# fredxia/openr

Measured on AMD Instinct MI355X. Metric: all-sources SPF solves/sec + GTEPS, 10k-node fabric, 1/2/4/8 MI355X, higher is better.
Workload: dtype u32; 1 GPU; fabric_full numOfSws=10000 (RoutingBenchmarkUtils.cpp:247-400, every pod wired); nodes=9976, directed_up_edges=232512, next_hop_rows=sliced

## Files before the change

### openr_amd/csrc/plan_host.cpp

```cpp
#include "plan_host.h"

#include <algorithm>
#include <map>
#include <numeric>
#include <utility>

namespace spfi {

PlanRows plan_rows(const GraphHost& g, const uint32_t* srcs, uint32_t n_src) {
  PlanRows r;
  r.row_of.assign(g.N, kInf);
  std::vector<uint32_t>& row_of = r.row_of;
  r.distinct = true;
  for (uint32_t i = 0; i < n_src; ++i) {
    if (row_of[srcs[i]] != kInf) r.distinct = false;
    else row_of[srcs[i]] = i;
  }
  bool closed = r.distinct;
  for (uint32_t i = 0; i < n_src && closed; ++i) {
    const uint32_t s = srcs[i];
    for (uint32_t j = g.nb_ptr[s]; j < g.nb_ptr[s + 1]; ++j) {
      const uint32_t x = g.nb_id[j];
      if (!g.ovl[x] && row_of[x] == kInf) {
        closed = false;
// ... 31 lines not shown
  l.nh_off.resize(n_src);
  l.words.resize(n_src);
  uint64_t off = 0;
  for (uint32_t i = 0; i < n_src; ++i) {
    const uint32_t k = g.nb_ptr[srcs[i] + 1] - g.nb_ptr[srcs[i]];
    l.words[i] = k;
    l.nh_off[i] = off;
    off += (uint64_t)k * (g.pitch / 32);
    l.wmax = std::max(l.wmax, (k + 31) / 32);
  }
  l.nh_total = off;
  return l;
}

NbRows plan_nb_rows(const GraphHost& g, const uint32_t* srcs, uint32_t n_src,
                    const std::vector<uint32_t>& row_of, uint64_t stride, size_t rows) {
  NbRows nb;
  nb.nb_row_off.resize(n_src);
  nb.nb_drained.assign(n_src, 0);
  const uint32_t dead = stride ? (uint32_t)(rows * stride) : kInf;
  nb.dead = dead;
  std::vector<uint32_t>& nb_row = nb.nb_row;
  for (uint32_t i = 0; i < n_src; ++i) {
    nb.nb_row_off[i] = (uint32_t)nb_row.size();
    for (uint32_t e = g.nb_ptr[srcs[i]]; e < g.nb_ptr[srcs[i] + 1]; ++e) {
      const uint32_t x = g.nb_id[e];
      const bool dr = g.ovl[x] != 0;
      nb_row.push_back(dr ? dead : stride ? (uint32_t)(row_of[x] * stride) : row_of[x]);
      nb.nb_drained[i] += dr;
    }
    const size_t k = nb_row.size() - nb.nb_row_off[i];
    nb_row.resize(nb.nb_row_off[i] + (k + 7) / 8 * 8 + 8, dead);
  }
  return nb;
}

ClassRows plan_class_rows(const GraphHost& g, const std::vector<uint32_t>& closure) {
  ClassRows cr;
  const std::vector<uint16_t>& cls = g.qt.cls;
  cr.fwd.assign(g.qt.n_cls, 0);
  for (uint32_t v = 0; v < g.N; ++v)
    if (!g.ovl[v]) cr.fwd[cls[v]] = 1;
  std::vector<uint32_t> src_of(g.qt.n_cls, kInf);
  cr.crow_of.resize(closure.size());
  for (size_t r = 0; r < closure.size(); ++r) {
    uint32_t& k = src_of[cls[closure[r]]];
    if (k == kInf) {
      k = (uint32_t)cr.csrc.size();
      cr.csrc.push_back(closure[r]);
    }
    cr.crow_of[r] = k;
  }
  return cr;
}

XcdLists plan_xcd_lists(const std::vector<uint32_t>& words, uint32_t runs) {
  XcdLists x;
  const uint32_t n_src = (uint32_t)words.size();
  if (runs == 0) {
    for (uint32_t i = 0; i < n_src; ++i) x.list[i % 8].push_back(i);
  } else {
    uint64_t total = 0, load[8] = {};
    for (uint32_t i = 0; i < n_src; ++i) total += words[i] + 1;
    const uint64_t target = std::max<uint64_t>(1, total / (8ull * runs));
    for (uint32_t i = 0; i < n_src;) {
      uint32_t e = i;
      uint64_t w = 0;
      while (e < n_src && w < target) w += words[e++] + 1;
      const int g = (int)(std::min_element(load, load + 8) - load);
      load[g] += w;
      for (uint32_t t = i; t < e; ++t) x.list[g].push_back(t);
      i = e;
    }
  }
  size_t most = 0;
  for (const auto& l : x.list) most = std::max(most, l.size());
  x.slot.assign(most * 8, kInf);
  for (int g = 0; g < 8; ++g)
    for (size_t t = 0; t < x.list[g].size(); ++t) x.slot[t * 8 + g] = x.list[g][t];
  x.slots = x.slot.size();
  if (x.slot.empty()) x.slot.push_back(kInf);
  return x;
}

uint32_t plan_sliced_unit(const std::vector<uint32_t>& words, uint32_t chunks, uint32_t n_cu) {
  uint64_t matches = 0;
  for (uint32_t k : words) matches += (uint64_t)k * chunks;
  return (uint32_t)std::min<uint64_t>(kSlUnit, std::max<uint64_t>(16, matches / (16ull * n_cu) / 8 * 8));
}

SlicedUnits plan_sliced_units(const std::vector<uint32_t> (&list)[8], const std::vector<uint32_t>& words,
                              const NbRows& nb, uint32_t chunks, uint32_t unit, int group) {
  SlicedUnits s;
  std::vector<uint32_t>& units = s.units;
  std::vector<uint32_t>& gtab = s.gtab;
  s.unit_off.assign(9, 0);
  const uint32_t dead = nb.dead;
  for (int g = 0; g < 8; ++g) {
    s.unit_off[g] = (uint32_t)(units.size() / 4);
    std::map<uint32_t, std::vector<uint8_t>> taken;
    std::map<std::vector<uint32_t>, std::vector<std::pair<uint32_t, uint32_t>>> shared;
    if (group) {
      std::map<std::vector<uint32_t>, std::vector<uint32_t>> seg;
      for (uint32_t i : list[g]) {
        const uint32_t k = words[i];
        if (!k) continue;
// ... 186 lines not shown
```

### openr_amd/csrc/plan_host.h

```cpp
#pragma once
#include <cstddef>
#include <cstdint>
#include <vector>

#include "graph_host.h"

namespace spfi {

constexpr uint32_t kEcmpRunsPerXcd = 64;
constexpr uint32_t kSlSlots = 8;
constexpr uint32_t kSlSat = 254;
constexpr uint32_t kSlGroup = 8;
constexpr uint32_t kSlSeg = 4;
constexpr uint32_t kSlUnit = 512;

struct PlanRows {
  bool distinct = false, direct = false;
  std::vector<uint32_t> closure, row_of, req_rows;
};
PlanRows plan_rows(const GraphHost& g, const uint32_t* srcs, uint32_t n_src);

struct NhLayout {
  std::vector<uint32_t> words;
  std::vector<uint64_t> nh_off;
  uint64_t nh_total = 0;
  uint32_t wmax = 1;
};
NhLayout plan_nh_layout(const GraphHost& g, const uint32_t* srcs, uint32_t n_src);

struct NbRows {
  std::vector<uint32_t> nb_row, nb_row_off, nb_drained;
  uint32_t dead = kInf;
};
NbRows plan_nb_rows(const GraphHost& g, const uint32_t* srcs, uint32_t n_src,
                    const std::vector<uint32_t>& row_of, uint64_t stride, size_t rows);

struct XcdLists {
  std::vector<uint32_t> list[8];
  std::vector<uint32_t> slot;
  size_t slots = 0;
};
XcdLists plan_xcd_lists(const std::vector<uint32_t>& words, uint32_t runs);

struct SlicedUnits {
  std::vector<uint32_t> units, unit_off, gtab;
  uint32_t max_xcd_units = 0;
};
SlicedUnits plan_sliced_units(const std::vector<uint32_t> (&list)[8], const std::vector<uint32_t>& words,
                              const NbRows& nb, uint32_t chunks, uint32_t unit, int group);
uint32_t plan_sliced_unit(const std::vector<uint32_t>& words, uint32_t chunks, uint32_t n_cu);

struct ClassRows {
  std::vector<uint32_t> csrc, crow_of;
  std::vector<uint8_t> fwd;
};
ClassRows plan_class_rows(const GraphHost& g, const std::vector<uint32_t>& closure);

struct DepthCache {
  std::vector<uint32_t> ecc;
  uint64_t ecc_epoch = ~0ull;
  uint32_t dbound = 0;
  uint64_t dbound_epoch = ~0ull;
  struct Memo {
    uint64_t sell_ver;
    std::vector<uint8_t> ovl;
    uint32_t dbound;
  };
  std::vector<Memo> memo;
};
const std::vector<uint32_t>& ecc_estimate(const GraphHost& g, DepthCache* m);
std::vector<uint32_t> plan_depth_order(const std::vector<uint32_t>& closure, const std::vector<uint32_t>& ecc);
uint32_t depth_bound(const GraphHost& g, DepthCache* m);

}
```

### openr_amd/csrc/spf_engine.hip

```cpp
#include <hip/hip_runtime.h>

#include <algorithm>
#include <chrono>
#include <cstdarg>
#include <cstdio>
#include <cstdlib>
#include <cstring>
#include <map>
#include <memory>
#include <mutex>
#include <numeric>
#include <string>
#include <type_traits>
#include <unordered_map>
#include <vector>

#include "engine_internal.h"
#include "wave_ops.h"

namespace spfi {

thread_local std::string g_err;

spf_status fail(spf_ctx* c, spf_status st, const char* fmt, ...) {
// ... 961 lines not shown
      uint32_t k[kQChunk];
#pragma unroll
      for (uint32_t j = 0; j < kQChunk; ++j) k[j] = vcol[j * q_nvp + r];
      uint64_t acc = 0;
#pragma unroll
      for (uint32_t j = 0; j < kQChunk; ++j) acc |= CFc[k[j]];
      if (acc) atomicOr(reinterpret_cast<unsigned long long*>(&QAc[vrow[r]]), acc);
    }
    for (uint32_t t = tid; t <= q_nc; t += kMsThreads) {
      CFn[t] = 0;
      QAn[t] = 0;
    }
    __syncthreads();
    uint64_t any = 0;
    for (uint32_t t0 = tid - lane; t0 < q_nc; t0 += kMsThreads) {
      const uint32_t t = t0 + lane;
      uint64_t nx = 0;
      if (t < q_nc) {
        const uint64_t v = VIS[t];
        nx = QAc[t] & ~v;
        if (nx) {
          VIS[t] = v | nx;
          if (fw[t]) CFn[t] = nx;
        }
      }
      any |= nx;
      for (uint64_t m = wave_or64(nx); m; m &= m - 1) {
        const uint32_t s = __ffsll((unsigned long long)m) - 1;
        if ((nx >> s) & 1ull) Dc[(size_t)(row0 + s) * cpitch + t] = (uint16_t)(L + 1);
      }
    }
    if (any) flag[L % 3] = 1;
    if (tid == 0) flag[(L + 1) % 3] = 0;
    __syncthreads();
    if (!flag[L % 3]) {
      last = L;
      break;
    }
  }
  if (tid == 0) atomicMax(maxd, last);
  for (uint32_t t0 = tid - lane; t0 < q_nc; t0 += kMsThreads) {
    const uint32_t t = t0 + lane;
    const uint64_t miss = t < q_nc ? ~VIS[t] & all : 0ull;
    for (uint64_t m = wave_or64(miss); m; m &= m - 1) {
      const uint32_t s = __ffsll((unsigned long long)m) - 1;
      if ((miss >> s) & 1ull) Dc[(size_t)(row0 + s) * cpitch + t] = 0xFFFFu;
    }
  }
  const uint32_t pw = cpitch - q_nc;
  for (uint32_t t = tid; t < nb * pw; t += kMsThreads)
    Dc[(size_t)(row0 + t / pw) * cpitch + q_nc + t % pw] = 0xFFFFu;
}

constexpr uint32_t kExThreads = 256;
constexpr uint32_t kExNodes = 4 * kExThreads;
constexpr uint32_t kExRows = 8;
__global__ __launch_bounds__(kExThreads) void expand_rows_kernel(
    const uint16_t* __restrict__ Dc, uint32_t cpitch, const uint32_t* __restrict__ crow_of,
    const uint32_t* __restrict__ closure, uint32_t rows, uint32_t rows_per,
    const uint16_t* __restrict__ q_cls, uint32_t q_nc, uint32_t N, uint32_t pitch, uint32_t npitch,
    uint32_t* __restrict__ D, uint8_t* __restrict__ Dn, uint32_t* __restrict__ S,
    const uint32_t* __restrict__ maxd) {
  extern __shared__ __attribute__((aligned(16))) unsigned char smem[];
  uint4* const T = reinterpret_cast<uint4*>(smem);
  uint32_t* const list = reinterpret_cast<uint32_t*>(T + kExNodes + 1);
  uint32_t* const cnt = list + kExNodes + 1;
  uint32_t* const map = cnt + 3;
  constexpr uint32_t kEmpty = 0xFFFFFFFFu, kClaimed = 0xFFFFFFFEu;

  const uint32_t tid = threadIdx.x, lane = tid & 63;
  const uint32_t cbase = blockIdx.x * kExNodes, v0 = cbase + tid * 4;
  const uint32_t r_begin = blockIdx.y * rows_per, r_end = min(rows, r_begin + rows_per);
  const uint32_t md = *maxd;
  const uint32_t P = (S && md < kSlSat) ? 32u - __clz(md + 1u) : 0u;
  const uint32_t wpm = pitch / 32;

  for (uint32_t t = tid; t < q_nc; t += kExThreads) map[t] = kEmpty;
  if (tid == 0) {
    *cnt = 1;
    T[0] = make_uint4(~0u, ~0u, ~0u, ~0u);
  }
  __syncthreads();
  uint32_t cl[4];
#pragma unroll
  for (int k = 0; k < 4; ++k) {
    cl[k] = v0 + k < N ? q_cls[v0 + k] : kEmpty;
    if (cl[k] != kEmpty && atomicCAS(&map[cl[k]], kEmpty, kClaimed) == kEmpty) {
      const uint32_t id = atomicAdd(cnt, 1u);
      list[id] = cl[k];
      map[cl[k]] = id;
    }
  }
  __syncthreads();
  const uint32_t n_loc = *cnt;
#pragma unroll
  for (int k = 0; k < 4; ++k) cl[k] = cl[k] != kEmpty ? map[cl[k]] : 0u;

  const uint32_t w = v0 / 32, pb = lane & 7u, nsh = 4u * pb;
  const bool d_live = D && v0 < pitch, n_live = Dn && v0 < npitch, s_live = pb < P && w < wpm;
  for (uint32_t r0 = r_begin; r0 < r_end; r0 += kExRows) {
    __syncthreads();
    for (uint32_t lc = 1 + tid; lc < n_loc; lc += kExThreads) {
      const uint32_t gc = list[lc];
      uint32_t x[kExRows];
#pragma unroll
      for (uint32_t j = 0; j < kExRows; ++j)
        x[j] = r0 + j < r_end ? Dc[(size_t)crow_of[r0 + j] * cpitch + gc] : 0xFFFFu;
      T[lc] = make_uint4(x[0] | x[1] << 16, x[2] | x[3] << 16, x[4] | x[5] << 16, x[6] | x[7] << 16);
    }
    __syncthreads();
    uint4 t[4];
#pragma unroll
    for (int k = 0; k < 4; ++k) t[k] = T[cl[k]];
#pragma unroll
    for (uint32_t j = 0; j < kExRows; ++j) {
      const uint32_t r = r0 + j;
      if (r >= r_end) break;
      uint32_t d[4];
#pragma unroll
      for (int k = 0; k < 4; ++k) {
        const uint32_t pair = j / 2 == 0 ? t[k].x : j / 2 == 1 ? t[k].y : j / 2 == 2 ? t[k].z : t[k].w;
        d[k] = (uint32_t)(int32_t)(int16_t)(pair >> (16 * (j & 1)));
      }
      const uint32_t self = closure[r] - v0;
      if (closure[r] - cbase < kExNodes) {
#pragma unroll
        for (int k = 0; k < 4; ++k) d[k] = self == (uint32_t)k ? 0u : d[k];
      }
      if (d_live) {
        typedef uint32_t u32x4 __attribute__((ext_vector_type(4)));
        const u32x4 o = {d[0], d[1], d[2], d[3]};
        __builtin_nontemporal_store(o, reinterpret_cast<u32x4*>(D + (size_t)r * pitch + v0));
      }
      if (n_live) {
        uint32_t b = 0;
#pragma unroll
        for (int k = 0; k < 4; ++k) b |= (d[k] == kInf ? 0xFFu : min(d[k], 254u)) << (8 * k);
        __builtin_nontemporal_store(b, reinterpret_cast<uint32_t*>(Dn + (size_t)r * npitch + v0));
      }
      if (P) {
        uint32_t mine = 0;
        for (uint32_t b = 0; b < P; ++b) {
          uint32_t nib = ((d[0] >> b) & 1u) | ((d[1] >> b) & 1u) << 1 | ((d[2] >> b) & 1u) << 2 |
                         ((d[3] >> b) & 1u) << 3;
          nib <<= nsh;
          nib |= (uint32_t)__builtin_amdgcn_update_dpp(0u, nib, 0xB1, 0xf, 0xf, true);
          nib |= (uint32_t)__builtin_amdgcn_update_dpp(0u, nib, 0x4E, 0xf, 0xf, true);
          nib |= (uint32_t)__builtin_amdgcn_update_dpp(0u, nib, 0x104, 0xf, 0x5, true) |
                 (uint32_t)__builtin_amdgcn_update_dpp(0u, nib, 0x114, 0xf, 0xa, true);
          mine = pb == b ? nib : mine;
        }
        if (s_live) S[(size_t)r * kSlSlots * wpm + (size_t)w * P + pb] = mine;
      }
    }
  }
}

template <int P>
struct Planes {
  uint32_t v[P];
};

typedef uint32_t u32x3 __attribute__((ext_vector_type(3)));
typedef uint32_t u32x4 __attribute__((ext_vector_type(4)));

template <int N>
__device__ __forceinline__ void bload(uint32_t* d, __amdgpu_buffer_rsrc_t r, uint32_t voff,
                                      uint32_t soff) {
  if constexpr (N >= 4) {
    const u32x4 a = __builtin_amdgcn_raw_buffer_load_b128(r, (int)voff, (int)soff, 0);
    d[0] = a.x, d[1] = a.y, d[2] = a.z, d[3] = a.w;
    if constexpr (N > 4) bload<N - 4>(d + 4, r, voff + 16, soff);
  } else if constexpr (N == 3) {
    const u32x3 a = __builtin_amdgcn_raw_buffer_load_b96(r, (int)voff, (int)soff, 0);
    d[0] = a.x, d[1] = a.y, d[2] = a.z;
  } else if constexpr (N == 2) {
    const u32x2 a = __builtin_amdgcn_raw_buffer_load_b64(r, (int)voff, (int)soff, 0);
    d[0] = a.x, d[1] = a.y;
  } else {
    d[0] = __builtin_amdgcn_raw_buffer_load_b32(r, (int)voff, (int)soff, 0);
  }
}

#ifndef SPF_SL_STORE_AUX
#define SPF_SL_STORE_AUX 2
#endif
constexpr int kSlStoreAux = SPF_SL_STORE_AUX;
template <int P, bool WEIGHTED = false, int U = (P <= 4 ? 4 : 2)>
__device__ __forceinline__ void sliced_pass(__amdgpu_buffer_rsrc_t rs, __amdgpu_buffer_rsrc_t ro,
                                            uint32_t wpm, uint32_t srow,
                                            const uint32_t* __restrict__ offs, uint32_t k,
                                            uint32_t jb, uint32_t w, bool live,
                                            const uint32_t* __restrict__ wts = nullptr) {
  const uint32_t wpb = w * P * 4;
  Planes<P> sv;
  bload<P>(sv.v, rs, wpb, srow * kSlSlots * wpm * 4);
  uint32_t t[P];
  uint32_t ones = ~0u, zeros = ~0u, borrow = ~0u;
#pragma unroll
  for (int b = 0; b < P; ++b) {
    const uint32_t x = sv.v[b];
    ones &= x;
    zeros &= ~x;
    t[b] = WEIGHTED ? x : x ^ borrow;
    borrow &= ~x;
  }
  const uint32_t valid = ~(ones | zeros);
// ... 326 lines not shown
      if (PASS) {
        const unsigned long long key = ((unsigned long long)du << 32) | r;
        uint32_t p = base + n;
        while (p > base) {
          const unsigned long long pk = pred_key[p - 1];
          if (pk < key) break;
          pred_key[p] = pk;
          pred_edge[p] = (uint32_t)pk;
          --p;
        }
        pred_key[p] = key;
        pred_edge[p] = r;
      }
      ++n;
    }
  }
  if (!PASS) cnt_or_ptr[v] = n;
}


size_t sssp_lds_bytes(uint32_t N, uint32_t pitch, uint32_t big, bool q16) {
  const uint32_t bm_words = (N + 31) / 32;
  size_t b = 4ull * pitch + 4ull * bm_words + 4ull * C_NWORDS + 4ull * big;
  b += (q16 ? 2ull : 4ull) * N;
  return (b + 15) & ~size_t(15);
}

size_t msbfs_lds_bytes(uint32_t N, bool db = false) {
  return 8ull * (N + 1) * (db ? 2 : 1) + 4ull * (4 * kMsBatch + 5);
}

bool ms_double_buffer(const spf_ctx* c) {
  const char* e = std::getenv("SPF_MSBFS_DB");
  if (e && e[0] == '0') return false;
  const size_t n_col = c->sell_ptr.back();
  return msbfs_lds_bytes(c->N) + 2ull * n_col > kMaxLds && msbfs_lds_bytes(c->N, true) <= kMaxLds;
}

size_t msbfs_q_lds_bytes(uint32_t N, uint32_t n_cls, uint32_t n_vrow) {
  const size_t nvp = (n_vrow + 7u) & ~7u;
  return 32ull * (n_cls + 1) + 2ull * (1 + kQChunk) * nvp + 4ull * (4 * kMsBatch + 5) + ((N + 3u) & ~3u);
}

bool quotient_allowed(const spf_ctx* c) {
  if (c->N > kMsMaxNodes || ms_own(c->N) > (uint32_t)kQMaxOwn) return false;
  const char* e = std::getenv("SPF_QUOTIENT");
  return !(e && e[0] == '0');
}

size_t class_bfs_lds_bytes(uint32_t n_cls, uint32_t n_vrow) {
  const size_t nvp = (n_vrow + 7u) & ~7u, nc1 = (n_cls + 2u) & ~1u;
  return 40ull * nc1 + 2ull * (1 + kQChunk) * nvp + 16 + ((n_cls + 15u) & ~15u);
}
size_t expand_lds_bytes(uint32_t n_cls) { return 20ull * (kExNodes + 1) + 12 + 4ull * n_cls + 16; }

uint32_t spread_batch(const spf_ctx* c, uint32_t rows, uint32_t full) {
  const uint32_t rounds = (rows + full * c->n_cu - 1) / (full * c->n_cu);
  return std::min<uint32_t>(full, (rows + rounds * c->n_cu - 1) / (rounds * c->n_cu));
}

uint32_t ms_batch(const spf_ctx* c, uint32_t rows, bool knob = true) {
  if (const char* e = knob ? std::getenv("SPF_MSBFS_BATCH") : nullptr) {
    const int b = atoi(e);
    if (b >= 1 && b <= (int)kMsBatch) return (uint32_t)b;
  }
  return spread_batch(c, rows, kMsBatch);
}

uint32_t planes_batch(const spf_ctx* c, uint32_t rows, bool ordered) {
  return ordered ? kPlBatch : spread_batch(c, rows, kPlBatch);
}

size_t planes_lds_bytes(uint32_t own) { return 8ull * own * kMsThreads + 4ull * (kPlBatch + 4); }

}

namespace spfi {

bool use_quotient(const spf_ctx* c) {
  const spf_ctx::Quotient& q = c->qt;
  if (!quotient_allowed(c) || q.stale || q.n_cls == 0 || 2 * q.n_edge > c->nb_id.size()) return false;
  return msbfs_q_lds_bytes(c->N, q.n_cls, q.n_vrow) <= kMaxLds;
}

bool plan_has_narrow(const spf_plan* p) {
  return !p->exact && !p->big && p->narrow && !p->sdirect && (p->d_Dn.p || p->cls);
}

bool use_planes(const spf_ctx* c) {
  if (c->N > 10 * (uint32_t)kMsThreads || c->sell4.empty()) return false;
  if (const char* e = std::getenv("SPF_MSBFS")) return e[0] == 'p';
  return c->sell_ptr.back() <= 8ull * c->N;
}

spf_status launch_sssp(spf_ctx* c, const uint32_t* rows_src, uint32_t rows, bool hop,
                       const uint32_t* ign, uint32_t* D, hipStream_t s, const uint32_t* wt,
                       const uint8_t* ovl, uint8_t* Dn, const uint32_t* redo) {
  if (!wt) wt = c->d_wt.p;
  if (!ovl) ovl = c->d_ovl.p;
  const uint32_t N = c->N, pitch = c->pitch, bm_words = (N + 31) / 32;
  const bool q16 = N <= 65535;
  const size_t lds = sssp_lds_bytes(N, pitch, c->big_nodes, q16);
  const bool unit = hop || c->max_metric == 1;
  uint32_t threads = lds > kMaxLds / 3 ? 1024u : lds > kMaxLds / 6 ? 512u : 256u;
  if (const char* e = std::getenv("SPF_SSSP_THREADS")) threads = (uint32_t)atoi(e);
  const dim3 g(rows);
#define SSSP_LAUNCH(QT, U, TH)                                                            \
// ... 219 lines not shown
  else if (own == 4) msbfs_launch<4>(c, rows_src, rows, D, Dn, maxd, d_from, s);
  else if (own == 8) msbfs_launch<8>(c, rows_src, rows, D, Dn, maxd, d_from, s);
  else if (own == 10) msbfs_launch<10>(c, rows_src, rows, D, Dn, maxd, d_from, s);
  else if (own == 12) msbfs_launch<12>(c, rows_src, rows, D, Dn, maxd, d_from, s);
  else msbfs_launch<16>(c, rows_src, rows, D, Dn, maxd, d_from, s);
  HIP_TRY(c, hipGetLastError());
  return SPF_OK;
}

template <bool NARROW>
spf_status launch_ecmp(spf_ctx* c, spf_plan* p, const uint8_t* Dn, const uint32_t* D, bool hop,
                       uint32_t* d_nh, hipStream_t s) {
  const uint32_t per_block = kEcmpChunk * kEcmpWaves;
  const uint32_t chunks = (c->N + per_block - 1) / per_block;
  const uint32_t nb = chunks * (uint32_t)p->slots;
  const uint32_t weighted = NARROW && !hop && !c->unit ? 1u : 0u;
  hipLaunchKernelGGL((ecmp_kernel<NARROW>), dim3(nb), dim3(kEcmpThreads), 0, s, Dn, c->npitch, D,
                     c->pitch, c->N, p->d_srcs.p, p->d_row_of.p, c->d_nb_ptr.p, c->d_nb_id.p,
                     c->d_nb_w.p, p->d_nb_row.p, p->d_nb_row_off.p, p->d_nb_drained.p, p->dead,
                     hop ? 1u : 0u, weighted,
                     p->d_nh_off.p, d_nh, chunks, p->d_slot_src.p);
  HIP_TRY(c, hipGetLastError());
  return SPF_OK;
}

spf_status launch_sliced(spf_ctx* c, spf_plan* p, const uint32_t* D, bool hop, uint32_t* d_nh,
                         hipStream_t s) {
  const uint32_t wpm = c->pitch / 32;
  const uint32_t rows = (uint32_t)p->closure.size();
  const uint64_t words = (uint64_t)rows * wpm;
  const uint32_t sb = (uint32_t)std::min<uint64_t>((words + 255) / 256, 16ull * c->n_cu);
  hipLaunchKernelGGL(slice_rows_kernel, dim3(std::max(sb, 1u)), dim3(256), 0, s, p->d_Dn.p, c->npitch,
                     rows, wpm, p->d_maxd.p, p->d_S.p, p->expand ? const_cast<uint32_t*>(D) : nullptr,
                     c->pitch);
  HIP_TRY(c, hipGetLastError());
  return SPF_OK;
}

spf_status launch_ecmp_sliced(spf_ctx* c, spf_plan* p, const uint32_t* D, bool hop, uint32_t* d_nh,
                              hipStream_t s) {
  const uint32_t blocks = 8 * std::max(1u, (p->max_xcd_units + kEcmpWaves - 1) / kEcmpWaves);
  hipLaunchKernelGGL(ecmp_sliced_kernel, dim3(blocks), dim3(kEcmpThreads), 0, s, p->d_S.p,
                     p->d_maxd.p, D, c->pitch, p->d_srcs.p, p->d_row_of.p,
                     c->d_nb_ptr.p, c->d_nb_id.p, c->d_nb_w.p, p->d_nb_row.p, p->d_nb_row_off.p,
                     p->d_nb_drained.p, p->dead, hop ? 1u : 0u, p->d_nh_off.p, d_nh,
                     reinterpret_cast<const uint4*>(p->d_units.p), p->d_unit_off.p, p->d_gtab.p,
                     (uint32_t)(p->d_S.n * 4), p->sdirect ? kTeamPlanes : 0u, p->mp ? 1u : 0u);
  HIP_TRY(c, hipGetLastError());
  return SPF_OK;
}

bool class_rows_fit(const spf_ctx* c) {
  return use_quotient(c) && class_bfs_lds_bytes(c->qt.n_cls, c->qt.n_vrow) <= kMaxLds &&
         expand_lds_bytes(c->qt.n_cls) <= kMaxLds;
}

spf_status launch_class_bfs(spf_ctx* c, spf_plan* p, hipStream_t s) {
  const uint32_t bs = ms_batch(c, p->cls_k);
  hipLaunchKernelGGL(class_bfs_kernel, dim3((p->cls_k + bs - 1) / bs), dim3(kMsThreads),
                     class_bfs_lds_bytes(c->qt.n_cls, c->qt.n_vrow), s, c->d_qcls.p, c->d_qtab.p,
                     c->qt.n_cls, c->qt.n_vrow, p->d_csrc.p, p->cls_k, bs, p->d_cfwd.p, p->d_Dc.p,
                     p->cls_pitch, p->d_maxd.p);
  HIP_TRY(c, hipGetLastError());
  return SPF_OK;
}

spf_status launch_expand(spf_ctx* c, spf_plan* p, uint32_t* D, uint8_t* Dn, uint32_t* S,
                         hipStream_t s) {
  const uint32_t rows = (uint32_t)p->closure.size();
  const uint32_t span = std::max(D ? c->pitch : 0u, Dn ? c->npitch : 0u);
  const uint32_t chunks = std::max(1u, (span + kExNodes - 1) / kExNodes);
  const uint32_t ranges = std::max(1u, 8 * c->n_cu / chunks);
  const uint32_t rows_per = ((rows + ranges - 1) / ranges + kExRows - 1) / kExRows * kExRows;
  hipLaunchKernelGGL(expand_rows_kernel, dim3(chunks, (rows + rows_per - 1) / rows_per),
                     dim3(kExThreads), expand_lds_bytes(c->qt.n_cls), s, p->d_Dc.p, p->cls_pitch,
                     p->d_crow_of.p, p->d_closure.p, rows, rows_per, c->d_qcls.p, c->qt.n_cls, c->N,
                     c->pitch, c->npitch, D, Dn, S, p->d_maxd.p);
  HIP_TRY(c, hipGetLastError());
  return SPF_OK;
}

struct PlanKnobs {
  int narrow = -1;
  int big = -1;
  bool pl_order = true;
  bool wsliced = true;
  bool expand = false;
  bool sdirect = true;
  bool class_rows = true;
  int64_t ecmp_runs = -1;
  int64_t sliced_unit = -1;
  int sliced_group = 2;
};

PlanKnobs plan_knobs() {
  auto first = [](const char* name) {
    const char* e = std::getenv(name);
    return e ? (int)(unsigned char)e[0] : -1;
  };
  auto number = [](const char* name) {
    const char* e = std::getenv(name);
    return e ? (int64_t)(uint32_t)atoi(e) : -1;
  };
  PlanKnobs k;
  const int nw = first("SPF_NARROW"), big = first("SPF_BIG");
  k.narrow = nw < 0 ? -1 : nw == '0' ? 0 : nw == '1' ? 1 : 2;
  k.big = big == '0' ? 0 : big == '1' ? 1 : -1;
  k.pl_order = first("SPF_PL_ORDER") != '0';
  k.wsliced = first("SPF_WSLICED") != '0';
  k.expand = first("SPF_EXPAND") == '1';
  k.sdirect = first("SPF_SDIRECT") != '0';
  k.class_rows = first("SPF_CLASS_ROWS") != '0';
  k.ecmp_runs = number("SPF_ECMP_RUNS");
  k.sliced_unit = number("SPF_SLICED_UNIT");
  if (const char* e = std::getenv("SPF_SLICED_GROUP")) k.sliced_group = atoi(e);
  return k;
}

bool plan_debug() {
  static const bool on = std::getenv("SPF_PLAN_DEBUG") != nullptr;
  return on;
}

bool use_narrow(const spf_ctx* c, const spf_plan* p, const PlanKnobs& kn) {
  if (kn.narrow >= 0) return kn.narrow != 0;
  if (use_planes(c)) return true;
  uint64_t nb = 0;
  for (uint32_t i = 0; i < p->n_src; ++i) nb += p->words[i];
  return nb >= 8ull * p->n_src;
// ... 296 lines not shown
  return SPF_OK;
}

spf_status spf_plan_traffic_phases(const spf_plan* p, uint64_t* bytes) {
  if (!p || !bytes) return SPF_E_INVALID;
  uint64_t* bfs_bytes = &bytes[0];
  uint64_t* ecmp_bytes = &bytes[2];
  bytes[1] = 0;
  const spf_ctx* c = p->ctx;
  const uint64_t N = c->N, E = c->E, rows = p->closure.size();
  uint64_t bfs = 0;
  if (p->big) {
    *bfs_bytes = rows * (4ull * (N + 1) + 12ull * E + N + 4ull * c->pitch) + 4ull * p->nh_total;
    *ecmp_bytes = 0;
    return SPF_OK;
  }
  if (p->exact) {
    const uint64_t lab = (p->flags & SPF_FLAG_DIST64) ? 8ull : 4ull;
    *bfs_bytes = rows * (4ull * (N + 1) + 12ull * E + N + 17ull * N + lab * c->pitch) +
                 4ull * p->nh_total;
    *ecmp_bytes = 0;
    return SPF_OK;
  }
  if (p->tm_G) {
    const uint64_t batches = (rows + p->tm_bs - 1) / p->tm_bs;
    const bool direct = p->prefix && !p->direct && p->narrow;
    const uint64_t wbytes = 4ull * (c->pitch / 32);
    bfs = batches * (8ull * c->sell_ptr.back() + N) + (direct ? p->n_src : rows) * c->pitch * 4ull +
          (p->sdirect ? rows * kTeamPlanes * wbytes : p->narrow ? rows * c->npitch : 0ull);
  } else if (p->cls) {
    const uint64_t bs = ms_batch(c, p->cls_k, false);
    const uint64_t groups = (p->cls_k + bs - 1) / bs;
    bfs = groups * (2ull * (c->qt.cls.size() + c->qt.tab.size()) + c->qt.n_cls) +
          2ull * p->cls_k * p->cls_pitch;
  } else if (p->ms) {
    const bool planes = use_planes(c);
    const uint64_t bs = planes ? planes_batch(c, (uint32_t)rows, false) : ms_batch(c, (uint32_t)rows, false);
    const uint64_t groups = (rows + bs - 1) / bs;
    const uint64_t n_slices = c->sell_ptr.size() - 1;
    const uint64_t csr = planes ? 8ull * c->sell4_ptr.back() + 4ull * (n_slices + 1)
                         : use_quotient(c) ? 2ull * (c->qt.cls.size() + c->qt.tab.size())
                                           : 4ull * c->sell_ptr.back() + 4ull * (n_slices + 1);
    bfs = groups * (csr + N) + (p->expand ? 0ull : rows * c->pitch * 4ull) +
          (p->narrow ? rows * c->npitch : 0ull);
  } else if (p->mp) {
    const uint64_t S = mssp_sources(c);
    const uint64_t groups = (rows + S - 1) / S;
    bfs = groups * (4ull * c->sell_ptr.back() + 4ull * c->sell_ptr.size() + 4ull * (N + 1) + N) +
          rows * (4ull * c->pitch + (p->narrow ? c->npitch : 0ull));
  } else {
    bfs = rows * (4ull * (N + 1) + 8ull * E + N + 4ull * c->pitch + (p->narrow ? c->npitch : 0ull));
  }
  *bfs_bytes = bfs;
  const uint64_t cls_expand = p->cls ? 2ull * p->cls_k * p->cls_pitch + 2ull * N + rows * 4ull * c->pitch +
                                           (p->keep_narrow ? rows * c->npitch : 0ull)
                                     : 0ull;
  bytes[1] = cls_expand;
  if (p->sliced && p->nh_total) {
    const uint64_t wbytes = 4ull * (c->pitch / 32);
    if (p->sdirect) {
      *ecmp_bytes = rows * kTeamPlanes * wbytes + 4ull * p->nh_total;
      return SPF_OK;
    }
    uint32_t md = 0;
    HIP_TRY(p->ctx, hipMemcpy(&md, p->d_maxd.p, 4, hipMemcpyDeviceToHost));
    const uint64_t expand = p->expand ? rows * 4ull * c->pitch : 0ull;
    if (md < kSlSat) {
      const uint64_t P = 32u - __builtin_clz(md + 1u);
      bytes[1] = p->cls ? cls_expand + rows * P * wbytes : rows * c->npitch + rows * P * wbytes + expand;
      *ecmp_bytes = rows * P * wbytes + 4ull * p->nh_total;
    } else {
      bytes[1] = p->cls ? cls_expand : expand ? rows * c->npitch + expand : 0ull;
      *ecmp_bytes = rows * 4ull * c->pitch + 4ull * p->nh_total;
    }
    return SPF_OK;
  }
  const uint64_t row_bytes = p->narrow ? c->npitch : 4ull * c->pitch;
  *ecmp_bytes = p->nh_total ? rows * row_bytes + 4ull * p->nh_total : 0ull;
  return SPF_OK;
}

spf_status spf_plan_nh_layout(const spf_plan* p, uint64_t* nh_off, uint32_t* words) {
  if (!p) return SPF_E_INVALID;
  for (uint32_t i = 0; i < p->n_src; ++i) {
    if (nh_off) nh_off[i] = p->nh_off[i];
    if (words) words[i] = p->words[i];
  }
  return SPF_OK;
}

spf_status spf_plan_execute(spf_plan* p, uint32_t* d_dist, uint32_t* d_nh, void* stream) {
  if (!p) return fail(nullptr, SPF_E_INVALID, "spf_plan_execute: NULL plan");
  spf_ctx* c = p->ctx;
  if (!c->loaded) return fail(c, SPF_E_STATE, "graph no longer loaded");
  if (!d_dist || (p->nh_total && !d_nh))
    return fail(c, SPF_E_INVALID, "spf_plan_execute: NULL output buffer");
  if (p->shape != c->shape)
    return fail(c, SPF_E_STATE, "graph reloaded since the plan was created: recreate it");
  if (p->layout != c->layout) {
    for (uint32_t i = 0; i < p->n_src; ++i)
      if (c->nb_ptr[p->srcs[i] + 1] - c->nb_ptr[p->srcs[i]] != p->words[i])
        return fail(c, SPF_E_STATE, "source %u's distinct neighbours changed since the plan was "
                                    "created (its next-hop layout): recreate it", p->srcs[i]);
    p->layout = c->layout;
  }
  if (p->epoch != c->epoch || (p->tm_G && c->team_off) || (p->cls && !use_quotient(c))) {
    const spf_status st = build_plan(c, p);
    if (st != SPF_OK) return st;
  }
// ... 366 lines not shown
```

Measured before the change: 50.69 million solves/s.

## Restructure expand kernel: full class-table staging, double-buffered row groups, occupancy-sized grid

The expand kernel no longer builds a per-block local class map with LDS atomics over a fixed node chunk. Each workgroup now stages the whole class table for 8 rows into LDS, loading it with vectorized reads, and walks row groups with a double-buffered prefetch of the next group. Waves stride over 256-node pieces. The grid is sized from the occupancy API so workgroups persist over row groups, and block size rises to 1024 threads. This should cut redundant Dc gathers and atomic setup per block, but it caps the class count by LDS size and adds an occupancy query on the host.

```diff
diff --git a/openr_amd/csrc/plan_host.cpp b/openr_amd/csrc/plan_host.cpp
--- a/openr_amd/csrc/plan_host.cpp
+++ b/openr_amd/csrc/plan_host.cpp
@@ -107,6 +107,24 @@
     cr.crow_of[r] = k;
   }
   return cr;
+}
+
+ExpandGrid plan_expand_grid(uint32_t rows, uint32_t span, uint32_t resident) {
+  ExpandGrid eg;
+  eg.groups = (rows + kExRows - 1) / kExRows;
+  eg.pieces = (span + kExPiece - 1) / kExPiece;
+  resident = std::max(1u, resident);
+  eg.pps = std::max(1u, eg.pieces);
+  if (eg.groups >= resident) {
+    eg.gper = (eg.groups + resident - 1) / resident;
+    eg.wgs = (eg.groups + eg.gper - 1) / eg.gper;
+  } else {
+    eg.wgs = std::max(1u, eg.groups);
+    const uint32_t want = std::min(eg.pps, resident / eg.wgs);
+    eg.pps = (eg.pps + want - 1) / want;
+    eg.splits = (std::max(1u, eg.pieces) + eg.pps - 1) / eg.pps;
+  }
+  return eg;
 }
 
 XcdLists plan_xcd_lists(const std::vector<uint32_t>& words, uint32_t runs) {
diff --git a/openr_amd/csrc/plan_host.h b/openr_amd/csrc/plan_host.h
--- a/openr_amd/csrc/plan_host.h
+++ b/openr_amd/csrc/plan_host.h
@@ -56,6 +56,15 @@
 };
 ClassRows plan_class_rows(const GraphHost& g, const std::vector<uint32_t>& closure);
 
+constexpr uint32_t kExRows = 8;
+constexpr uint32_t kExPiece = 256;
+struct ExpandGrid {
+  uint32_t groups = 0, pieces = 0;
+  uint32_t wgs = 1, gper = 1;
+  uint32_t splits = 1, pps = 1;
+};
+ExpandGrid plan_expand_grid(uint32_t rows, uint32_t span, uint32_t resident);
+
 struct DepthCache {
   std::vector<uint32_t> ecc;
   uint64_t ecc_epoch = ~0ull;
diff --git a/openr_amd/csrc/spf_engine.hip b/openr_amd/csrc/spf_engine.hip
--- a/openr_amd/csrc/spf_engine.hip
+++ b/openr_amd/csrc/spf_engine.hip
@@ -1037,107 +1037,128 @@
     Dc[(size_t)(row0 + t / pw) * cpitch + q_nc + t % pw] = 0xFFFFu;
 }
 
-constexpr uint32_t kExThreads = 256;
-constexpr uint32_t kExNodes = 4 * kExThreads;
-constexpr uint32_t kExRows = 8;
+#ifndef SPF_EX_THREADS
+#define SPF_EX_THREADS 1024
+#endif
+constexpr uint32_t kExThreads = SPF_EX_THREADS;
+constexpr uint32_t kExWaves = kExThreads / 64;
+constexpr uint32_t kExMaxCls = 8 * kExThreads - 8;
+__host__ __device__ constexpr uint32_t ex_entries(uint32_t q_nc) { return (q_nc + 8u) & ~7u; }
+
+__device__ __forceinline__ void ex_stage_load(uint4 (&x)[kExRows], const uint16_t* __restrict__ Dc,
+                                              uint32_t cpitch, const uint32_t* __restrict__ crow_of,
+                                              uint32_t r0, uint32_t rows, uint32_t o) {
+#pragma unroll
+  for (uint32_t j = 0; j < kExRows; ++j) {
+    x[j] = make_uint4(~0u, ~0u, ~0u, ~0u);
+    if (r0 + j < rows && 8u * o < cpitch)
+      x[j] = *reinterpret_cast<const uint4*>(Dc + (size_t)crow_of[r0 + j] * cpitch + 8u * o);
+  }
+}
+
+__device__ __forceinline__ void ex_stage_write(uint4* __restrict__ T, const uint4 (&x)[kExRows], uint32_t o) {
+#pragma unroll
+  for (uint32_t i = 0; i < 8; ++i) {
+    uint32_t h[kExRows];
+#pragma unroll
+    for (uint32_t j = 0; j < kExRows; ++j) {
+      const uint32_t w = i / 2 == 0 ? x[j].x : i / 2 == 1 ? x[j].y : i / 2 == 2 ? x[j].z : x[j].w;
+      h[j] = (i & 1u) ? w >> 16 : w & 0xFFFFu;
+    }
+    T[8u * o + i] = make_uint4(h[0] | h[1] << 16, h[2] | h[3] << 16, h[4] | h[5] << 16, h[6] | h[7] << 16);
+  }
+}
+
 __global__ __launch_bounds__(kExThreads) void expand_rows_kernel(
     const uint16_t* __restrict__ Dc, uint32_t cpitch, const uint32_t* __restrict__ crow_of,
-    const uint32_t* __restrict__ closure, uint32_t rows, uint32_t rows_per,
+    const uint32_t* __restrict__ closure, uint32_t rows, uint32_t gper, uint32_t pieces, uint32_t pps,
     const uint16_t* __restrict__ q_cls, uint32_t q_nc, uint32_t N, uint32_t pitch, uint32_t npitch,
     uint32_t* __restrict__ D, uint8_t* __restrict__ Dn, uint32_t* __restrict__ S,
     const uint32_t* __restrict__ maxd) {
   extern __shared__ __attribute__((aligned(16))) unsigned char smem[];
+  const uint32_t nT = ex_entries(q_nc);
   uint4* const T = reinterpret_cast<uint4*>(smem);
-  uint32_t* const list = reinterpret_cast<uint32_t*>(T + kExNodes + 1);
-  uint32_t* const cnt = list + kExNodes + 1;
-  uint32_t* const map = cnt + 3;
-  constexpr uint32_t kEmpty = 0xFFFFFFFFu, kClaimed = 0xFFFFFFFEu;
-
-  const uint32_t tid = threadIdx.x, lane = tid & 63;
-  const uint32_t cbase = blockIdx.x * kExNodes, v0 = cbase + tid * 4;
-  const uint32_t r_begin = blockIdx.y * rows_per, r_end = min(rows, r_begin + rows_per);
+
+  const uint32_t tid = threadIdx.x, lane = tid & 63, wave = tid >> 6;
+  const uint32_t groups = (rows + kExRows - 1) / kExRows;
+  const uint32_t g_begin = blockIdx.x * gper, g_end = min(groups, g_begin + gper);
+  const uint32_t p_begin = blockIdx.y * pps, p_end = min(pieces, p_begin + pps);
   const uint32_t md = *maxd;
   const uint32_t P = (S && md < kSlSat) ? 32u - __clz(md + 1u) : 0u;
   const uint32_t wpm = pitch / 32;
-
-  for (uint32_t t = tid; t < q_nc; t += kExThreads) map[t] = kEmpty;
-  if (tid == 0) {
-    *cnt = 1;
-    T[0] = make_uint4(~0u, ~0u, ~0u, ~0u);
-  }
-  __syncthreads();
-  uint32_t cl[4];
-#pragma unroll
-  for (int k = 0; k < 4; ++k) {
-    cl[k] = v0 + k < N ? q_cls[v0 + k] : kEmpty;
-    if (cl[k] != kEmpty && atomicCAS(&map[cl[k]], kEmpty, kClaimed) == kEmpty) {
-      const uint32_t id = atomicAdd(cnt, 1u);
-      list[id] = cl[k];
-      map[cl[k]] = id;
-    }
-  }
-  __syncthreads();
-  const uint32_t n_loc = *cnt;
-#pragma unroll
-  for (int k = 0; k < 4; ++k) cl[k] = cl[k] != kEmpty ? map[cl[k]] : 0u;
-
-  const uint32_t w = v0 / 32, pb = lane & 7u, nsh = 4u * pb;
-  const bool d_live = D && v0 < pitch, n_live = Dn && v0 < npitch, s_live = pb < P && w < wpm;
-  for (uint32_t r0 = r_begin; r0 < r_end; r0 += kExRows) {
+  const bool stager = tid < nT / 8;
+  const uint32_t pb = lane & 7u, nsh = 4u * pb;
+
+  uint4 x[kExRows];
+  if (stager && g_begin < g_end) {
+    ex_stage_load(x, Dc, cpitch, crow_of, g_begin * kExRows, rows, tid);
+    ex_stage_write(T, x, tid);
+  }
+  for (uint32_t g = g_begin; g < g_end; ++g) {
+    const uint4* const cur = T + ((g - g_begin) & 1u) * nT;
     __syncthreads();
-    for (uint32_t lc = 1 + tid; lc < n_loc; lc += kExThreads) {
-      const uint32_t gc = list[lc];
-      uint32_t x[kExRows];
-#pragma unroll
-      for (uint32_t j = 0; j < kExRows; ++j)
-        x[j] = r0 + j < r_end ? Dc[(size_t)crow_of[r0 + j] * cpitch + gc] : 0xFFFFu;
-      T[lc] = make_uint4(x[0] | x[1] << 16, x[2] | x[3] << 16, x[4] | x[5] << 16, x[6] | x[7] << 16);
-    }
-    __syncthreads();
-    uint4 t[4];
-#pragma unroll
-    for (int k = 0; k < 4; ++k) t[k] = T[cl[k]];
-#pragma unroll
-    for (uint32_t j = 0; j < kExRows; ++j) {
-      const uint32_t r = r0 + j;
-      if (r >= r_end) break;
-      uint32_t d[4];
-#pragma unroll
-      for (int k = 0; k < 4; ++k) {
-        const uint32_t pair = j / 2 == 0 ? t[k].x : j / 2 == 1 ? t[k].y : j / 2 == 2 ? t[k].z : t[k].w;
-        d[k] = (uint32_t)(int32_t)(int16_t)(pair >> (16 * (j & 1)));
-      }
-      const uint32_t self = closure[r] - v0;
-      if (closure[r] - cbase < kExNodes) {
-#pragma unroll
-        for (int k = 0; k < 4; ++k) d[k] = self == (uint32_t)k ? 0u : d[k];
-      }
-      if (d_live) {
-        typedef uint32_t u32x4 __attribute__((ext_vector_type(4)));
-        const u32x4 o = {d[0], d[1], d[2], d[3]};
-        __builtin_nontemporal_store(o, reinterpret_cast<u32x4*>(D + (size_t)r * pitch + v0));
-      }
-      if (n_live) {
-        uint32_t b = 0;
-#pragma unroll
-        for (int k = 0; k < 4; ++k) b |= (d[k] == kInf ? 0xFFu : min(d[k], 254u)) << (8 * k);
-        __builtin_nontemporal_store(b, reinterpret_cast<uint32_t*>(Dn + (size_t)r * npitch + v0));
-      }
-      if (P) {
-        uint32_t mine = 0;
-        for (uint32_t b = 0; b < P; ++b) {
-          uint32_t nib = ((d[0] >> b) & 1u) | ((d[1] >> b) & 1u) << 1 | ((d[2] >> b) & 1u) << 2 |
-                         ((d[3] >> b) & 1u) << 3;
-          nib <<= nsh;
-          nib |= (uint32_t)__builtin_amdgcn_update_dpp(0u, nib, 0xB1, 0xf, 0xf, true);
-          nib |= (uint32_t)__builtin_amdgcn_update_dpp(0u, nib, 0x4E, 0xf, 0xf, true);
-          nib |= (uint32_t)__builtin_amdgcn_update_dpp(0u, nib, 0x104, 0xf, 0x5, true) |
-                 (uint32_t)__builtin_amdgcn_update_dpp(0u, nib, 0x114, 0xf, 0xa, true);
-          mine = pb == b ? nib : mine;
+    const bool more = stager && g + 1 < g_end;
+    if (more) ex_stage_load(x, Dc, cpitch, crow_of, (g + 1) * kExRows, rows, tid);
+    const uint32_t r0 = g * kExRows, nr = min(kExRows, rows - r0);
+    for (uint32_t pc = p_begin + wave; pc < p_end; pc += kExWaves) {
+      const uint32_t pbase = pc * kExPiece, v0 = pbase + lane * 4;
+      uint32_t cl[4];
+      if (v0 + 4 <= N) {
+        const uint2 c2 = *reinterpret_cast<const uint2*>(q_cls + v0);
+        cl[0] = c2.x & 0xFFFFu, cl[1] = c2.x >> 16, cl[2] = c2.y & 0xFFFFu, cl[3] = c2.y >> 16;
+      } else {
+#pragma unroll
+        for (int k = 0; k < 4; ++k) cl[k] = v0 + k < N ? q_cls[v0 + k] : q_nc;
+      }
+      uint4 t[4];
+#pragma unroll
+      for (int k = 0; k < 4; ++k) t[k] = cur[cl[k]];
+      const uint32_t w = v0 / 32;
+      const bool d_live = D && v0 < pitch, n_live = Dn && v0 < npitch, s_live = pb < P && w < wpm;
+#pragma unroll
+      for (uint32_t j = 0; j < kExRows; ++j) {
+        if (j >= nr) break;
+        const uint32_t r = r0 + j;
+        uint32_t d[4];
+#pragma unroll
+        for (int k = 0; k < 4; ++k) {
+          const uint32_t pair = j / 2 == 0 ? t[k].x : j / 2 == 1 ? t[k].y : j / 2 == 2 ? t[k].z : t[k].w;
+          d[k] = (uint32_t)(int32_t)(int16_t)(pair >> (16 * (j & 1)));
         }
-        if (s_live) S[(size_t)r * kSlSlots * wpm + (size_t)w * P + pb] = mine;
-      }
-    }
+        const uint32_t own = closure[r];
+        if (own - pbase < kExPiece) {
+          const uint32_t self = own - v0;
+#pragma unroll
+          for (int k = 0; k < 4; ++k) d[k] = self == (uint32_t)k ? 0u : d[k];
+        }
+        if (d_live) {
+          typedef uint32_t u32x4 __attribute__((ext_vector_type(4)));
+          const u32x4 o = {d[0], d[1], d[2], d[3]};
+          __builtin_nontemporal_store(o, reinterpret_cast<u32x4*>(D + (size_t)r * pitch + v0));
+        }
+        if (n_live) {
+          uint32_t b = 0;
+#pragma unroll
+          for (int k = 0; k < 4; ++k) b |= (d[k] == kInf ? 0xFFu : min(d[k], 254u)) << (8 * k);
+          __builtin_nontemporal_store(b, reinterpret_cast<uint32_t*>(Dn + (size_t)r * npitch + v0));
+        }
+        if (P) {
+          uint32_t mine = 0;
+          for (uint32_t b = 0; b < P; ++b) {
+            uint32_t nib = ((d[0] >> b) & 1u) | ((d[1] >> b) & 1u) << 1 | ((d[2] >> b) & 1u) << 2 |
+                           ((d[3] >> b) & 1u) << 3;
+            nib <<= nsh;
+            nib |= (uint32_t)__builtin_amdgcn_update_dpp(0u, nib, 0xB1, 0xf, 0xf, true);
+            nib |= (uint32_t)__builtin_amdgcn_update_dpp(0u, nib, 0x4E, 0xf, 0xf, true);
+            nib |= (uint32_t)__builtin_amdgcn_update_dpp(0u, nib, 0x104, 0xf, 0x5, true) |
+                   (uint32_t)__builtin_amdgcn_update_dpp(0u, nib, 0x114, 0xf, 0xa, true);
+            mine = pb == b ? nib : mine;
+          }
+          if (s_live) S[(size_t)r * kSlSlots * wpm + (size_t)w * P + pb] = mine;
+        }
+      }
+    }
+    if (more) ex_stage_write(T + ((g + 1 - g_begin) & 1u) * nT, x, tid);
   }
 }
 
@@ -1570,7 +1591,7 @@
   const size_t nvp = (n_vrow + 7u) & ~7u, nc1 = (n_cls + 2u) & ~1u;
   return 40ull * nc1 + 2ull * (1 + kQChunk) * nvp + 16 + ((n_cls + 15u) & ~15u);
 }
-size_t expand_lds_bytes(uint32_t n_cls) { return 20ull * (kExNodes + 1) + 12 + 4ull * n_cls + 16; }
+size_t expand_lds_bytes(uint32_t n_cls) { return 2ull * 16 * ex_entries(n_cls); }
 
 uint32_t spread_batch(const spf_ctx* c, uint32_t rows, uint32_t full) {
   const uint32_t rounds = (rows + full * c->n_cu - 1) / (full * c->n_cu);
@@ -1896,7 +1917,7 @@
 
 bool class_rows_fit(const spf_ctx* c) {
   return use_quotient(c) && class_bfs_lds_bytes(c->qt.n_cls, c->qt.n_vrow) <= kMaxLds &&
-         expand_lds_bytes(c->qt.n_cls) <= kMaxLds;
+         c->qt.n_cls <= kExMaxCls && expand_lds_bytes(c->qt.n_cls) <= kMaxLds;
 }
 
 spf_status launch_class_bfs(spf_ctx* c, spf_plan* p, hipStream_t s) {
@@ -1909,16 +1930,28 @@
   return SPF_OK;
 }
 
+uint32_t expand_resident(const spf_ctx* c) {
+  static size_t for_lds = 0;
+  static int per_cu = 0;
+  const size_t lds = expand_lds_bytes(c->qt.n_cls);
+  if (lds != for_lds) {
+    int n = 0;
+    if (hipOccupancyMaxActiveBlocksPerMultiprocessor(&n, expand_rows_kernel, (int)kExThreads, lds) != hipSuccess)
+      n = 0;
+    per_cu = std::max(1, n);
+    for_lds = lds;
+  }
+  return c->n_cu * (uint32_t)per_cu;
+}
+
 spf_status launch_expand(spf_ctx* c, spf_plan* p, uint32_t* D, uint8_t* Dn, uint32_t* S,
                          hipStream_t s) {
   const uint32_t rows = (uint32_t)p->closure.size();
-  const uint32_t span = std::max(D ? c->pitch : 0u, Dn ? c->npitch : 0u);
-  const uint32_t chunks = std::max(1u, (span + kExNodes - 1) / kExNodes);
-  const uint32_t ranges = std::max(1u, 8 * c->n_cu / chunks);
-  const uint32_t rows_per = ((rows + ranges - 1) / ranges + kExRows - 1) / kExRows * kExRows;
-  hipLaunchKernelGGL(expand_rows_kernel, dim3(chunks, (rows + rows_per - 1) / rows_per),
-                     dim3(kExThreads), expand_lds_bytes(c->qt.n_cls), s, p->d_Dc.p, p->cls_pitch,
-                     p->d_crow_of.p, p->d_closure.p, rows, rows_per, c->d_qcls.p, c->qt.n_cls, c->N,
+  const uint32_t span = std::max((D || S) ? c->pitch : 0u, Dn ? c->npitch : 0u);
+  const ExpandGrid eg = plan_expand_grid(rows, span, expand_resident(c));
+  hipLaunchKernelGGL(expand_rows_kernel, dim3(eg.wgs, eg.splits), dim3(kExThreads),
+                     expand_lds_bytes(c->qt.n_cls), s, p->d_Dc.p, p->cls_pitch, p->d_crow_of.p,
+                     p->d_closure.p, rows, eg.gper, eg.pieces, eg.pps, c->d_qcls.p, c->qt.n_cls, c->N,
                      c->pitch, c->npitch, D, Dn, S, p->d_maxd.p);
   HIP_TRY(c, hipGetLastError());
   return SPF_OK;
@@ -2321,9 +2354,13 @@
     bfs = rows * (4ull * (N + 1) + 8ull * E + N + 4ull * c->pitch + (p->narrow ? c->npitch : 0ull));
   }
   *bfs_bytes = bfs;
-  const uint64_t cls_expand = p->cls ? 2ull * p->cls_k * p->cls_pitch + 2ull * N + rows * 4ull * c->pitch +
-                                           (p->keep_narrow ? rows * c->npitch : 0ull)
-                                     : 0ull;
+  uint64_t cls_expand = 0;
+  if (p->cls) {
+    const ExpandGrid eg = plan_expand_grid((uint32_t)rows, std::max(c->pitch, p->keep_narrow ? c->npitch : 0u),
+                                           expand_resident(c));
+    cls_expand = eg.splits * rows * 2ull * p->cls_pitch + (uint64_t)eg.groups * 2ull * N +
+                 rows * 4ull * c->pitch + (p->keep_narrow ? rows * c->npitch : 0ull);
+  }
   bytes[1] = cls_expand;
   if (p->sliced && p->nh_total) {
     const uint64_t wbytes = 4ull * (c->pitch / 32);
```

New measurement: 56.38 million solves/s, median of 6. 1.11x the previous value.
